# google/yggdrasil-decision-forests

Measured on NVIDIA H100. Metric: GBT boosting iters/sec, 10M rows x 200 num feats, higher is better.
Workload: dtype int64 fixed-point sums (q24 gradients), f64 split scores

## Files before the change

### include/ygg_b200.h

```cpp
#ifndef YGG_B200_H_
#define YGG_B200_H_

#include <stdint.h>

#ifdef __cplusplus
extern "C" {
#endif

#define YGG_ABI_VERSION 3

enum ygg_status {
  YGG_OK = 0,
  YGG_ERR_INVALID_ARGUMENT = 1,
  YGG_ERR_NO_DEVICE = 2,
  YGG_ERR_CUDA = 3,
  YGG_ERR_UNIMPLEMENTED = 4,
  YGG_ERR_CANCELLED = 5,
  YGG_ERR_IO = 6
};

enum ygg_loss {
  YGG_LOSS_BINOMIAL_LOG_LIKELIHOOD = 0,
  YGG_LOSS_SQUARED_ERROR = 1,
  YGG_LOSS_MULTINOMIAL_LOG_LIKELIHOOD = 2
// ... 150 lines not shown
int ygg_num_candidate_attributes(int32_t num_features, int32_t loss, int32_t num_candidate_attributes,
                                 float num_candidate_attributes_ratio, int32_t* k);
uint64_t ygg_candidate_key(uint32_t random_seed, int32_t tree, int32_t node, int32_t feature);
int ygg_gbt_set_candidate_sampling(ygg_gbt* h, int32_t num_candidate_attributes, float num_candidate_attributes_ratio);

int ygg_gbt_set_dart(ygg_gbt* h, float dropout_rate);
int ygg_gbt_get_dart_weights(ygg_gbt* h, float* out, int32_t capacity, int32_t* n);
int ygg_gbt_get_dart_dropped(ygg_gbt* h, int32_t iter, int32_t* out, int32_t capacity, int32_t* n);

int ygg_gbt_get_tree(ygg_gbt* h, int32_t iter, ygg_node* out, int32_t capacity, int32_t* n_nodes);
int ygg_gbt_get_category_set(ygg_gbt* h, int32_t iter, int32_t node, uint32_t* words, int32_t capacity, int32_t* n_words);
int ygg_gbt_train_loss(ygg_gbt* h, int32_t iter, float* loss, float* secondary);
int ygg_gbt_get_predictions(ygg_gbt* h, float* out, int64_t n);
int ygg_gbt_predict(ygg_gbt* h, const ygg_dataset* ds, float* out, int64_t n);

int ygg_gbt_set_predictions(ygg_gbt* h, const float* pred, int64_t n);

int ygg_tree_train_on_gradients(ygg_gbt* h, const float* gradients, const float* hessians,
                                ygg_node* out, int32_t capacity, int32_t* n_nodes);

enum ygg_hist_mode {
  YGG_HIST_ROOT_SUM = 0,
  YGG_HIST_PACKED = 1,
  YGG_HIST_SHARED = 2,
  YGG_HIST_HIST2 = 3,
  YGG_HIST_SEGMENTED = 4,
};
typedef struct ygg_hist_plan {
  int32_t mode;
  int32_t group;
  union {
    int32_t hist2_tiles;
    int32_t root_lanes;
  };
  int32_t chunk_blocks;
  int32_t slot_window;
  int32_t grid;
} ygg_hist_plan;
int ygg_debug_hist_plan(const ygg_gbt* h, int32_t level, ygg_hist_plan* out);
int ygg_debug_level_histogram(ygg_gbt* h, int32_t level, const ygg_hist_plan* plan, const float* gradients,
                              const float* second, const int32_t* slot_of_row, int32_t n_slots, uint64_t* out_sum,
                              uint32_t* out_cnt, uint64_t* out_second, float* out_scales);

int ygg_debug_wide_histogram(ygg_gbt* h, int32_t n_slots, uint64_t* out_sum, uint32_t* out_cnt, uint64_t* out_second);

int ygg_debug_capture_candidates(ygg_gbt* h, int32_t enabled);
typedef struct ygg_level_node {
  int32_t node;
  int32_t candidate;
  int32_t derived;
  int32_t reserved;
  int64_t num_examples;
} ygg_level_node;
typedef struct ygg_candidate {
  int32_t found;
  float score;
  int32_t threshold_bin;
  int32_t lo, hi;
  int32_t num_pos_examples;
  float threshold_value;
  uint32_t cat_mask[8];
} ygg_candidate;
int ygg_debug_level_candidates(ygg_gbt* h, int32_t level, int32_t capacity, ygg_level_node* nodes, ygg_candidate* cands,
                               uint32_t* sets, int32_t set_words, int32_t* n_nodes, float* scales);
int ygg_debug_level_tried(ygg_gbt* h, int32_t level, int32_t capacity, uint8_t* tried, int32_t* first_node, int32_t* n_nodes);

// ... 15 lines not shown
```

### yggdrasil-decision-forests_b200/_capi.py

```python
import ctypes as C
import os

import numpy as np

from . import _build

_LIB = None


class YggError(RuntimeError):
    def __init__(self, code, msg):
        super().__init__(f"[ygg status {code}] {msg}")
        self.code = code


class GbtConfig(C.Structure):
    _fields_ = [
        ("abi_version", C.c_int32), ("loss", C.c_int32), ("num_trees", C.c_int32),
        ("shrinkage", C.c_float), ("max_depth", C.c_int32), ("min_examples", C.c_int32),
        ("in_split_min_examples_check", C.c_int32), ("use_hessian_gain", C.c_int32),
        ("l1_regularization", C.c_float), ("l2_regularization", C.c_float),
        ("l2_regularization_categorical", C.c_float), ("clamp_leaf_logit", C.c_float),
        ("hessian_split_score_subtract_parent", C.c_int32), ("random_seed", C.c_uint32),
        ("subsample", C.c_float), ("validation_ratio", C.c_float),
# ... 2 lines not shown
        ("num_classes", C.c_int32), ("candidate_shuffle", C.c_int32), ("rng_words_consumed", C.c_uint32),
        ("split_jobs_draw_seeds", C.c_int32), ("growing_strategy", C.c_int32), ("max_num_nodes", C.c_int32),
        ("goss_alpha", C.c_float), ("goss_beta", C.c_float),
    ]


NODE_DTYPE = np.dtype([
    ("feature", "<i4"), ("threshold_bin", "<i4"), ("na_value", "<i4"), ("depth", "<i4"),
    ("neg_child", "<i4"), ("pos_child", "<i4"), ("split_score", "<f4"), ("leaf_value", "<f4"),
    ("num_examples", "<i8"), ("num_pos_examples", "<i8"), ("stat", "<f8", (3,)),
    ("condition_type", "<i4"), ("threshold_value", "<f4"), ("cat_mask", "<u4", (8,)),
])
assert NODE_DTYPE.itemsize == 112

FEATURE_DISCRETIZED_NUMERICAL = 0
FEATURE_CATEGORICAL = 1
FEATURE_NUMERICAL = 2

LEVEL_NODE_DTYPE = np.dtype([("node", "<i4"), ("candidate", "<i4"), ("derived", "<i4"), ("reserved", "<i4"),
                             ("num_examples", "<i8")])
assert LEVEL_NODE_DTYPE.itemsize == 24
CANDIDATE_DTYPE = np.dtype([("found", "<i4"), ("score", "<f4"), ("threshold_bin", "<i4"), ("lo", "<i4"), ("hi", "<i4"),
                            ("num_pos_examples", "<i4"), ("threshold_value", "<f4"), ("cat_mask", "<u4", (8,))])
assert CANDIDATE_DTYPE.itemsize == 60

HIST_ROOT_SUM, HIST_PACKED, HIST_SHARED, HIST2, HIST_SEGMENTED = 0, 1, 2, 3, 4


class HistPlan(C.Structure):
    _fields_ = [("mode", C.c_int32), ("group", C.c_int32), ("hist2_tiles", C.c_int32), ("chunk_blocks", C.c_int32),
                ("slot_window", C.c_int32), ("grid", C.c_int32)]

    root_lanes = property(lambda self: self.hist2_tiles, lambda self, v: setattr(self, "hist2_tiles", v))

    def __repr__(self):
        return "HistPlan(%s)" % ", ".join("%s=%d" % (k, getattr(self, k)) for k, _ in self._fields_)

ALLGATHER_FN = C.CFUNCTYPE(C.c_int, C.c_void_p, C.c_void_p, C.c_void_p, C.c_int64, C.c_void_p)
ALLREDUCE_FN = C.CFUNCTYPE(C.c_int, C.c_void_p, C.c_void_p, C.c_int64, C.c_int32, C.c_int32, C.c_void_p)
REDUCESCATTER_FN = C.CFUNCTYPE(C.c_int, C.c_void_p, C.c_void_p, C.c_int64, C.c_int32, C.c_int32, C.c_void_p)

EXPORTS = [
    "ygg_abi_version", "ygg_last_error", "ygg_device_count", "ygg_dataset_create",
    "ygg_dataset_set_feature_types", "ygg_dataset_destroy", "ygg_dataset_num_rows", "ygg_dataset_num_features",
    "ygg_gbt_config_init", "ygg_gbt_create", "ygg_gbt_destroy", "ygg_gbt_set_labels_i32",
    "ygg_gbt_set_labels_f32", "ygg_gbt_set_weights_f32", "ygg_gbt_set_validation_weights_f32", "ygg_gbt_set_feature_shard", "ygg_gbt_set_row_shard", "ygg_gbt_set_row_shard_scatter", "ygg_feature_shard",
    "ygg_merge_shard_best", "ygg_gbt_initial_prediction",
    "ygg_gbt_train", "ygg_gbt_train_timed", "ygg_gbt_step", "ygg_gbt_sync", "ygg_gbt_num_trees", "ygg_gbt_get_tree",
    "ygg_gbt_train_loss", "ygg_gbt_get_predictions", "ygg_gbt_set_predictions", "ygg_gbt_predict",
    "ygg_tree_train_on_gradients", "ygg_debug_hist_plan", "ygg_debug_level_histogram", "ygg_partition_rows",
    "ygg_gbt_set_profiling", "ygg_gbt_get_profile", "ygg_gbt_save_ydf",
    "ygg_discretize_boundaries", "ygg_discretize_encode", "ygg_model_write_ydf",
    "ygg_validation_split_mask", "ygg_dataset_split_rows", "ygg_gbt_set_validation_i32",
    "ygg_gbt_set_validation_f32", "ygg_gbt_validation_loss", "ygg_gbt_num_iterations", "ygg_gbt_final_validation",
    "ygg_gen_discretized_boundaries", "ygg_dataset_builder_create", "ygg_dataset_builder_add_numerical",
    "ygg_dataset_builder_add_numerical_async", "ygg_dataset_builder_get_numerical",
    "ygg_dataset_builder_add_bins", "ygg_dataset_builder_finish", "ygg_dataset_builder_destroy",
    "ygg_dataset_get_bins", "ygg_dataset_set_bucket_values", "ygg_gbt_tie_stats", "ygg_gbt_set_tie_rng_position",
    "ygg_gbt_best_split_window_bytes", "ygg_gbt_set_best_split_window", "ygg_comm_window_create",
    "ygg_comm_unique_id", "ygg_comm_create", "ygg_comm_destroy", "ygg_comm_allreduce", "ygg_comm_allgather", "ygg_comm_reducescatter",
    "ygg_dataset_set_wide_column", "ygg_dataset_get_wide_column", "ygg_debug_wide_histogram",
    "ygg_dataset_set_wide_categorical_column", "ygg_gbt_get_category_set",
    "ygg_dataset_set_numerical_column", "ygg_dataset_get_numerical_column",
    "ygg_debug_capture_candidates", "ygg_debug_level_candidates",
    "ygg_num_candidate_attributes", "ygg_candidate_key", "ygg_gbt_set_candidate_sampling", "ygg_debug_level_tried",
    "ygg_gbt_set_dart", "ygg_gbt_get_dart_weights", "ygg_gbt_get_dart_dropped",
# ... 737 lines not shown
```

### yggdrasil-decision-forests_b200/csrc/ygg_engine.cu

```cuda
#include <algorithm>
#include <mutex>
#include <random>
#include <cmath>
#include <cstdarg>
#include <cstdio>
#include <cstdlib>
#include <cstring>
#include <limits>
#include <map>
#include <queue>
#include <string>
#include <thread>
#include <vector>

#include <cuda_runtime.h>
#include <cub/device/device_radix_sort.cuh>
#include <cub/device/device_scan.cuh>
#include <nvtx3/nvToolsExt.h>

#include "../../include/ygg_b200.h"
#include "ygg_internal.h"
#include "../../include/ygg_b200_model.h"
#include "ygg_kernels.cuh"
#include "ygg_wide.cuh"
// ... 64 lines not shown
  return YGG_OK;
}
template <typename T>
int dev_alloc_plain(T** p, size_t count) {
  YGG_CUDA(cudaMalloc(reinterpret_cast<void**>(p), std::max<size_t>(count, 1) * sizeof(T)));
  return YGG_OK;
}
inline void dev_free(void* p) {
  if (p != nullptr) cudaFreeAsync(p, nullptr);
}

struct ProfileSlot {
  double ms = 0;
  int64_t launches = 0;
};

}


struct LossRec {
  double loss_sum;
  unsigned long long correct;
};

enum ShardMode { kShardNone = 0, kShardFeatures = 1, kShardRows = 2 };

struct HistLaunch {
  int mode;
  int G, S;
  int chunk, grid;
  int window, passes;
  int FL, T;
  int SL;
  int RL;
};

struct ygg_gbt {
  ygg_dataset* ds = nullptr;
  ygg_gbt_config cfg{};
  cudaStream_t stream = nullptr;
  bool has_labels = false;
  uint8_t* d_label_u8 = nullptr;
  float* d_label_f32 = nullptr;
  float initial_prediction = 0.f;
  float* d_pred = nullptr;
  float* d_g = nullptr;
  float* d_h = nullptr;
  uint32_t* d_q24 = nullptr;
  uint32_t* d_hq24 = nullptr;
  uint2* d_act = nullptr;
  uint32_t* d_act_h = nullptr;
  int32_t* d_act_count = nullptr;
  int32_t* d_act_sub = nullptr;
  uint32_t* d_root_cnt = nullptr;
  bool root_cnt_valid = false;
  int n_blocks = 0;
  uint16_t* d_node_of_row = nullptr;
  DeviceState* d_st = nullptr;
  LevelDesc* d_levels = nullptr;
  Family* d_fam[2] = {nullptr, nullptr};
  int32_t* d_slot_node[2] = {nullptr, nullptr};
  NodeRec* d_nodes_all = nullptr;
  NodeRec* d_nodes_scratch = nullptr;
  int tree_capacity = 0;
  unsigned long long* d_hist_sum[2] = {nullptr, nullptr};
  uint32_t* d_hist_cnt[2] = {nullptr, nullptr};
// ... 304 lines not shown
    YGG_RETURN_IF_ERROR(check_launch("k_sub_counts"));
  }
  uint32_t* d_max = *d_sub + static_cast<size_t>(n_subs) * f_count * kMaxBins;
  YGG_CUDA(cudaMemset(d_max, 0, sizeof(uint32_t)));
  const int subs_per_chunk = chunk_blocks / kSubBlocks;
  const int n_chunks = (n_subs + subs_per_chunk - 1) / subs_per_chunk;
  k_chunk_max<<<dim3(n_chunks, f_count), 256>>>(*d_sub, n_subs, subs_per_chunk, d_max);
  YGG_CUDA(cudaMemcpy(out_max, d_max, sizeof(uint32_t), cudaMemcpyDeviceToHost));
  return YGG_OK;
}

int raise_hist_smem_caps_once(int device) {
  static std::mutex mu;
  static std::vector<char> done;
  std::lock_guard<std::mutex> lock(mu);
  if (static_cast<int>(done.size()) <= device) done.resize(device + 1, 0);
  if (done[device]) return YGG_OK;
  size_t budget = 0;
  YGG_RETURN_IF_ERROR(hist_smem_budget(device, &budget));
  auto set_cap = [](size_t bytes) {
    return [bytes](auto kern) -> int {
      YGG_CUDA(cudaFuncSetAttribute(kern, cudaFuncAttributeMaxDynamicSharedMemorySize, static_cast<int>(bytes)));
      return YGG_OK;
    };
  };
  for (const bool hess : {false, true})
    for (const int mode : {kHistRootSum, kHistPacked, kHistShared})
      for (const bool multi : {false, true}) YGG_RETURN_IF_ERROR(for_hist_kernel(hess, mode, set_cap(budget), multi));
  const auto cap2 = set_cap(kHist2SmemBudget);
  YGG_RETURN_IF_ERROR(cap2(k_hist2<32, true>)); YGG_RETURN_IF_ERROR(cap2(k_hist2<32, false>));
  YGG_RETURN_IF_ERROR(cap2(k_hist2<16, true>)); YGG_RETURN_IF_ERROR(cap2(k_hist2<16, false>));
  YGG_RETURN_IF_ERROR(cap2(k_hist2<8, true>)); YGG_RETURN_IF_ERROR(cap2(k_hist2<8, false>));
  YGG_RETURN_IF_ERROR(set_cap(seg_smem_bytes(64))(k_hist_seg<32, 2>));
  YGG_RETURN_IF_ERROR(set_cap(seg_smem_bytes(32))(k_hist_seg<32, 1>));
  YGG_RETURN_IF_ERROR(set_cap(seg_smem_bytes(16))(k_hist_seg<16, 1>));
  YGG_RETURN_IF_ERROR(set_cap(seg_smem_bytes(8))(k_hist_seg<8, 1>));
  YGG_CUDA(cudaFuncSetAttribute(k_hist_seg<32, 2>, cudaFuncAttributePreferredSharedMemoryCarveout, cudaSharedmemCarveoutMaxShared));
  YGG_CUDA(cudaFuncSetAttribute(k_hist_seg<32, 1>, cudaFuncAttributePreferredSharedMemoryCarveout, cudaSharedmemCarveoutMaxShared));
  YGG_CUDA(cudaFuncSetAttribute(k_hist_seg<16, 1>, cudaFuncAttributePreferredSharedMemoryCarveout, cudaSharedmemCarveoutMaxShared));
  YGG_CUDA(cudaFuncSetAttribute(k_hist_seg<8, 1>, cudaFuncAttributePreferredSharedMemoryCarveout, cudaSharedmemCarveoutMaxShared));
  YGG_RETURN_IF_ERROR(set_cap(kRootSmemBytes)(k_hist_root_rows));
  done[device] = 1;
  return YGG_OK;
}

int configure_launches(ygg_gbt* h) {
  (void)cudaGetLastError();
  const bool hh = hist_hess(h);
  size_t budget = 0;
  YGG_RETURN_IF_ERROR(hist_smem_budget(h->ds->device, &budget));
  YGG_RETURN_IF_ERROR(raise_hist_smem_caps_once(h->ds->device));
  const int f_count = h->hist_f_end - h->hist_f_begin;
  const int n_blocks = static_cast<int>(h->ds->n_pad / kBlockRows);
  const int kSubBlocks = sub_blocks_of(h);
  const double min_items = 1.0, min_items2 = 0.9;
  auto choose_chunk = [&](int n_fgroups, int grid, int step, double need) {
    const int max_c = std::max(step, kHistMaxChunkBlocks / step * step);
    const int min_chunks = std::max(1, (n_blocks + max_c - 1) / max_c);
    int best = max_c;
    double best_score = -1;
    for (int nc = min_chunks; nc <= std::max(min_chunks, n_blocks); nc++) {
      const int c = std::min(max_c, ((n_blocks + nc - 1) / nc + step - 1) / step * step);
      const int real_nc = (n_blocks + c - 1) / c;
      const double per_cta = static_cast<double>(real_nc) * n_fgroups / grid;
      if (per_cta > 8.0 && nc > min_chunks) break;
      const double fill = static_cast<double>(n_blocks) / (static_cast<double>(real_nc) * c);
      const double eff = per_cta / std::ceil(per_cta) * fill;
      const double score = eff + (per_cta >= need ? 0.08 : 0.0);
      if (score > best_score + 1e-9) { best_score = score; best = c; }
    }
// ... 6 lines not shown
  for (int l = 0; l < h->num_levels; l++) {
    HistLaunch& pl = h->hist_plan[l];
    pl.mode = hh ? kHistShared : (l == 0 && !sampling(h)) ? kHistRootSum : kHistPacked;
    int S = level_slot_bound(h, l);
    pl.window = 0;
    pl.passes = 1;
    if (hist_smem_bytes(1, S, hh, pl.mode) > budget) {
      if (S > 254)
        return set_error(YGG_ERR_UNIMPLEMENTED, "max_depth=%d needs %d histogram slots at level %d; the active lists carry 8-bit slots",
                         h->cfg.max_depth, S, l);
      int s_pass = 1;
      while (hist_smem_bytes(1, 2 * s_pass + 1, hh, pl.mode) <= budget) s_pass *= 2;
      pl.window = s_pass;
      pl.passes = (S + s_pass - 1) / s_pass;
      S = s_pass + 1;
    }
    int G = 1;
    while (G < 8 && G < f_count && hist_smem_bytes(G + 1, S, hh, pl.mode) <= budget) G++;
    pl.G = G;
    pl.S = S;
    pl.grid = h->ds->num_sms;
    pl.FL = pl.T = 0;
    if (want_hist2 && !hh && S <= 2 && (l > 0 || pl.mode == kHistRootSum)) {
      int FL = 32;
      while (FL > 8 && FL / 2 >= 4 * n_groups) FL /= 2;
      int T = 2;
      if (hist2_smem_bytes(FL, S, T, l == 0) > kHist2SmemBudget) T = 1;
      if (hist2_smem_bytes(FL, S, T, l == 0) <= kHist2SmemBudget) { pl.FL = FL; pl.T = T; }
    }
    const bool packed = pl.mode == kHistPacked || (pl.FL > 0 && l > 0);
    const int n_fgroups = pl.FL > 0 ? (n_groups + pl.FL / 4 - 1) / (pl.FL / 4) : (f_count + G - 1) / G;
    pl.chunk = choose_chunk(n_fgroups, pl.grid, packed ? kSubBlocks : 1, pl.FL > 0 ? min_items2 : min_items);
    pl.SL = 0;
    pl.RL = 0;
    khist_plan[l] = pl;
    const int S_level = level_slot_bound(h, l);
    if (!hh && l > 0 && pl.mode == kHistPacked && pl.FL == 0 && S_level >= seg_min_slots(f_count, h->ds->n)) {
      int SL = 32;
      while (SL > 8 && SL / 2 >= f_count) SL /= 2;
      pl.SL = SL;
      pl.G = 1;
      pl.S = S_level;
      pl.window = 0;
      pl.passes = 1;
      pl.grid = h->ds->num_sms * kSegMinBlocks;
      pl.chunk = std::min(std::max(kSubBlocks, kHistMaxChunkBlocks / kSubBlocks * kSubBlocks),
                          (n_blocks + kSubBlocks - 1) / kSubBlocks * kSubBlocks);
    }
  }
  {
    std::map<int, uint32_t> max_of_chunk;
    uint32_t* d_sub = nullptr;
    int status = YGG_OK;
    for (int l = 0; l < h->num_levels && status == YGG_OK; l++) {
      HistLaunch& pl = h->hist_plan[l];
      if (pl.mode != kHistPacked && (pl.FL == 0 || l == 0)) continue;
      int chunk = pl.chunk;
      while (chunk >= kSubBlocks) {
        auto it = max_of_chunk.find(chunk);
        if (it == max_of_chunk.end()) {
          uint32_t m = 0;
          status = chunk_max_count(h, chunk, &d_sub, &m);
          if (status != YGG_OK) break;
          it = max_of_chunk.emplace(chunk, m).first;
        }
        if (it->second <= kPackedMaxUpdates) break;
        const int smaller = static_cast<int>(static_cast<double>(chunk) * 0.9 * kPackedMaxUpdates / it->second) / kSubBlocks * kSubBlocks;
        const int next = std::min(smaller, chunk - kSubBlocks);
        chunk = (next < kSubBlocks && chunk > kSubBlocks) ? kSubBlocks : next;
      }
      if (chunk < kSubBlocks) {
        if (pl.SL > 0) pl = khist_plan[l];
        pl.mode = kHistShared;
// ... 322 lines not shown
  h->d_hseg = nullptr; h->d_hseg_blk = nullptr; h->d_hseg_off = nullptr; h->d_hseg_piece = nullptr; h->d_hseg_meta = nullptr;
  h->d_hseg_temp = nullptr;
  h->hseg_temp_bytes = 0;
}
int ensure_seg_buffers(ygg_gbt* h) {
  if (h->d_hseg_temp != nullptr) return YGG_OK;
  const size_t ranges = static_cast<size_t>(kSegMaxSlots) * h->n_blocks;
  auto alloc_all = [&]() -> int {
    YGG_RETURN_IF_ERROR(dev_alloc(&h->d_hseg, static_cast<size_t>(h->ds->n_pad)));
    YGG_RETURN_IF_ERROR(dev_alloc(&h->d_hseg_blk, ranges));
    YGG_RETURN_IF_ERROR(dev_alloc(&h->d_hseg_off, ranges + 1));
    YGG_RETURN_IF_ERROR(dev_alloc(&h->d_hseg_piece, ranges + 1));
    YGG_RETURN_IF_ERROR(dev_alloc(&h->d_hseg_meta, 4));
    size_t temp_bytes = 0;
    YGG_CUDA(cub::DeviceScan::InclusiveSum(nullptr, temp_bytes, h->d_hseg_blk, h->d_hseg_blk, static_cast<int>(ranges)));
    char* temp = nullptr;
    YGG_RETURN_IF_ERROR(dev_alloc(&temp, temp_bytes));
    h->hseg_temp_bytes = temp_bytes;
    h->d_hseg_temp = temp;
    return YGG_OK;
  };
  const int st = alloc_all();
  if (st != YGG_OK) free_seg_buffers(h);
  return st;
}

int launch_hist_seg(ygg_gbt* h, int l, const LevelBuf& lb, const LevelDesc* levels, const HistLaunch& pl) {
  ygg_dataset* ds = h->ds;
  YGG_RETURN_IF_ERROR(ensure_bins_rows(ds));
  YGG_RETURN_IF_ERROR(ensure_seg_buffers(h));
  const int f_count = h->hist_f_end - h->hist_f_begin;
  const int n_chunks = (h->n_blocks + pl.chunk - 1) / pl.chunk;
  const int fpl = seg_lane_features(pl.SL, f_count);
  const int n_fg = seg_feature_groups(pl.SL, fpl, h->hist_f_begin, f_count);
  const int target_pieces = std::max(1, (kSegItemsPerCta * pl.grid + n_fg - 1) / n_fg);
  k_seg_count<<<std::min(h->n_blocks, ds->num_sms * 8), 256, 0, h->stream>>>(h->d_act, h->d_act_count, h->n_blocks, pl.S,
                                                                               levels, l, h->d_hseg_blk);
  YGG_RETURN_IF_ERROR(check_launch("k_seg_count"));
  YGG_CUDA(cub::DeviceScan::InclusiveSum(h->d_hseg_temp, h->hseg_temp_bytes, h->d_hseg_blk, h->d_hseg_blk, pl.S * h->n_blocks,
                                         h->stream));
  k_seg_ranges<<<1, kSegScanThreads, 0, h->stream>>>(h->d_hseg_blk, pl.S, h->n_blocks, pl.chunk, n_chunks, target_pieces,
                                                     h->d_hseg_off, h->d_hseg_piece, h->d_hseg_meta);
  YGG_RETURN_IF_ERROR(check_launch("k_seg_ranges"));
  k_seg_scatter<<<std::min(h->n_blocks, ds->num_sms * 8), 256, 0, h->stream>>>(h->d_act, h->d_act_count, h->n_blocks, pl.S, levels, l,
                                                               h->d_hseg_blk, h->d_hseg);
  YGG_RETURN_IF_ERROR(check_launch("k_seg_scatter"));
  SegParams sp{};
  sp.rows = ds->d_bins_rows; sp.row_bytes = static_cast<uint32_t>(seg_row_bytes(ds->F));
  sp.seg = h->d_hseg; sp.seg_off = h->d_hseg_off; sp.piece_start = h->d_hseg_piece; sp.meta = h->d_hseg_meta;
  sp.n_ranges = pl.S * n_chunks; sp.n_chunks = n_chunks;
  sp.f_begin = h->hist_f_begin; sp.f_count = f_count;
  sp.hist_sum = lb.sum; sp.hist_cnt = lb.cnt;
  sp.f_chunk = lb.f_chunk; sp.chunk_stride = static_cast<long long>(lb.chunk_u64);
  const size_t smem = seg_smem_bytes(pl.SL * fpl);
  if (fpl == 2) k_hist_seg<32, 2><<<pl.grid, kSegThreads, smem, h->stream>>>(sp);
  else if (pl.SL == 32) k_hist_seg<32, 1><<<pl.grid, kSegThreads, smem, h->stream>>>(sp);
  else if (pl.SL == 16) k_hist_seg<16, 1><<<pl.grid, kSegThreads, smem, h->stream>>>(sp);
  else k_hist_seg<8, 1><<<pl.grid, kSegThreads, smem, h->stream>>>(sp);
  h->launches_total += 5;
  return check_launch("k_hist_seg");
}

int launch_hist_root_rows(ygg_gbt* h, const LevelBuf& lb, const HistLaunch& pl) {
  ygg_dataset* ds = h->ds;
  YGG_RETURN_IF_ERROR(ensure_bins_rows(ds));
  RootRowsParams rp{};
  rp.rows = ds->d_bins_rows; rp.row_bytes = static_cast<uint32_t>(seg_row_bytes(ds->F));
  rp.q24 = h->d_q24; rp.act_count = h->d_act_count; rp.n_blocks = h->n_blocks; rp.chunk_blocks = pl.chunk;
  rp.f_begin = h->hist_f_begin; rp.f_count = h->hist_f_end - h->hist_f_begin;
  rp.hist_sum = lb.sum; rp.f_chunk = lb.f_chunk; rp.chunk_stride = static_cast<long long>(lb.chunk_u64);
  k_hist_root_rows<<<pl.grid, kRootThreads, kRootSmemBytes, h->stream>>>(rp);
  h->launches_total++;
  return check_launch("k_hist_root_rows");
}

int ensure_root_counts(ygg_gbt* h) {
  if (h->root_cnt_valid) return YGG_OK;
  const int f_count = h->hist_f_end - h->hist_f_begin;
  if (h->d_root_cnt) dev_free(h->d_root_cnt);
  h->d_root_cnt = nullptr;
  const LevelBuf lb = level_buf(h, 1, 1);
  const size_t padded = static_cast<size_t>(lb.W) * lb.f_chunk * kMaxBins;
  YGG_RETURN_IF_ERROR(dev_alloc(&h->d_root_cnt, padded));
  YGG_CUDA(cudaMemsetAsync(h->d_root_cnt, 0, padded * sizeof(uint32_t), h->stream));
  dim3 grid(std::max(1, h->ds->num_sms * 8 / std::max(1, f_count)), f_count);
  k_root_counts<<<grid, 256, 0, h->stream>>>(h->ds->d_bins, h->ds->n, h->ds->n_pad, f_count, h->hist_f_begin, h->d_root_cnt);
  h->launches_total++;
  YGG_RETURN_IF_ERROR(check_launch("k_root_counts"));
// ... 2444 lines not shown
  YGG_CUDA(cudaSetDevice(h->ds->device));
  (void)cudaGetLastError();
  YGG_RETURN_IF_ERROR(apply_pending(h));
  const int64_t n = h->ds->n;
  YGG_CUDA(cudaMemcpyAsync(h->d_g, gradients, n * sizeof(float), cudaMemcpyHostToDevice, h->stream));
  if (has_h(h)) YGG_CUDA(cudaMemcpyAsync(h->d_h, hessians, n * sizeof(float), cudaMemcpyHostToDevice, h->stream));
  const int root_candidate = (n >= h->cfg.min_examples && 1 < h->cfg.max_depth) ? 1 : 0;
  k_begin_iteration<<<1, 1, 0, h->stream>>>(h->d_st, h->d_levels, h->d_fam[0], h->d_slot_node[0], root_candidate);
  h->launches_total++;
  k_absmax<<<elementwise_grid(h), 256, 0, h->stream>>>(h->d_g, n, h->d_st);
  h->launches_total++;
  YGG_RETURN_IF_ERROR(check_launch("k_absmax"));
  h->scratch_tree = false;
  YGG_RETURN_IF_ERROR(grow_tree(h, h->d_nodes_scratch));
  if (h->cfg.growing_strategy == 1) YGG_RETURN_IF_ERROR(best_first_prune(h, h->d_nodes_scratch));
  YGG_RETURN_IF_ERROR(check_device_error(h));
  h->scratch_tree = true;
  std::vector<ygg_node> flat;
  YGG_RETURN_IF_ERROR(fetch_tree(h, h->d_nodes_scratch, &flat, true));
  *n_nodes = static_cast<int32_t>(flat.size());
  if (static_cast<int32_t>(flat.size()) > capacity) return set_error(YGG_ERR_INVALID_ARGUMENT, "capacity %d < %zu nodes", capacity, flat.size());
  std::memcpy(out, flat.data(), flat.size() * sizeof(ygg_node));
  return YGG_OK;
}

int ygg_debug_hist_plan(const ygg_gbt* h, int32_t level, ygg_hist_plan* out) {
  if (!h || !out) return set_error(YGG_ERR_INVALID_ARGUMENT, "null argument");
  if (level < 0 || level >= h->num_levels) return set_error(YGG_ERR_INVALID_ARGUMENT, "level %d outside [0, %d)", level, h->num_levels);
  const HistLaunch& pl = h->hist_plan[level];
  ygg_hist_plan p{};
  if (pl.FL > 0) {
    p.mode = YGG_HIST_HIST2; p.group = pl.FL; p.hist2_tiles = pl.T;
  } else if (pl.SL > 0) {
    p.mode = YGG_HIST_SEGMENTED; p.group = pl.SL;
  } else {
    p.mode = pl.mode == kHistRootSum ? YGG_HIST_ROOT_SUM : pl.mode == kHistPacked ? YGG_HIST_PACKED : YGG_HIST_SHARED;
    p.group = pl.G;
    p.root_lanes = pl.RL;
  }
  p.chunk_blocks = pl.chunk;
  p.slot_window = pl.window;
  p.grid = pl.grid;
  *out = p;
  return YGG_OK;
}

int ygg_debug_level_histogram(ygg_gbt* h, int32_t level, const ygg_hist_plan* plan, const float* gradients,
                              const float* second, const int32_t* slot_of_row, int32_t n_slots, uint64_t* out_sum,
                              uint32_t* out_cnt, uint64_t* out_second, float* out_scales) {
  if (!h || !gradients || !slot_of_row || !out_sum || !out_cnt || !out_scales) return set_error(YGG_ERR_INVALID_ARGUMENT, "null argument");
  if (level < 0 || level >= h->num_levels) return set_error(YGG_ERR_INVALID_ARGUMENT, "level %d outside [0, %d)", level, h->num_levels);
  if (n_slots < 1 || n_slots > 254) return set_error(YGG_ERR_INVALID_ARGUMENT, "n_slots=%d outside [1, 254] (8-bit slots)", n_slots);
  const bool hh = hist_hess(h);
  if (hh != (second != nullptr) || hh != (out_second != nullptr))
    return set_error(YGG_ERR_INVALID_ARGUMENT, hh ? "this handle keeps a second histogram plane: `second` and `out_second` are required"
                                                  : "this handle keeps no second histogram plane: `second` and `out_second` must be NULL");
  const float v_pow2 = hh ? (weighted(h) ? h->w_pow2 : h_pow2_of(h)) : 0.f;
  const int64_t n = h->ds->n;
  bool all_slot0 = true;
  for (int64_t r = 0; r < n; r++) {
    if (!std::isfinite(gradients[r])) return set_error(YGG_ERR_INVALID_ARGUMENT, "gradient of row %lld is not finite", static_cast<long long>(r));
    if (hh && !(second[r] >= 0.f && second[r] <= v_pow2))
      return set_error(YGG_ERR_INVALID_ARGUMENT, "second-plane value of row %lld outside [0, %g]", static_cast<long long>(r), v_pow2);
    if (slot_of_row[r] < -1 || slot_of_row[r] >= n_slots)
      return set_error(YGG_ERR_INVALID_ARGUMENT, "slot %d of row %lld outside [-1, %d)", slot_of_row[r], static_cast<long long>(r), n_slots);
    all_slot0 &= slot_of_row[r] == 0;
  }
  HistLaunch pl{};
  if (plan == nullptr) {
    pl = h->hist_plan[level];
    if (n_slots > level_slot_bound(h, level))
      return set_error(YGG_ERR_INVALID_ARGUMENT, "the plan of level %d holds %d slots, %d requested", level, level_slot_bound(h, level), n_slots);
  } else {
    const ygg_hist_plan& p = *plan;
    if (p.mode < YGG_HIST_ROOT_SUM || p.mode > YGG_HIST_SEGMENTED) return set_error(YGG_ERR_INVALID_ARGUMENT, "unknown mode %d", p.mode);
    const bool root_rows = p.mode == YGG_HIST_ROOT_SUM && p.root_lanes != 0;
    if (root_rows && p.root_lanes != kRootLanes)
      return set_error(YGG_ERR_INVALID_ARGUMENT, "root_lanes=%d: 0 (k_hist) or %d (k_hist_root_rows)", p.root_lanes, kRootLanes);
    const int max_chunk = root_rows ? kRootRowsMaxChunkBlocks : kHistMaxChunkBlocks;
    if (p.chunk_blocks < 1 || p.chunk_blocks > max_chunk)
      return set_error(YGG_ERR_INVALID_ARGUMENT, "chunk_blocks=%d outside [1, %d]", p.chunk_blocks, max_chunk);
    if (p.grid < 1 || p.grid > 65535) return set_error(YGG_ERR_INVALID_ARGUMENT, "grid=%d outside [1, 65535]", p.grid);
    if (p.slot_window < 0) return set_error(YGG_ERR_INVALID_ARGUMENT, "slot_window=%d", p.slot_window);
    pl.chunk = p.chunk_blocks; pl.grid = p.grid;
    if (p.mode == YGG_HIST_HIST2) {
      if (p.group != 8 && p.group != 16 && p.group != 32) return set_error(YGG_ERR_INVALID_ARGUMENT, "k_hist2: %d feature lanes (8, 16 or 32)", p.group);
      if (p.hist2_tiles != 1 && p.hist2_tiles != 2) return set_error(YGG_ERR_INVALID_ARGUMENT, "k_hist2: %d sub-tiles (1 or 2)", p.hist2_tiles);
      if (p.slot_window != 0) return set_error(YGG_ERR_INVALID_ARGUMENT, "k_hist2 has no multi-pass form");
      if (n_slots > 2) return set_error(YGG_ERR_INVALID_ARGUMENT, "k_hist2 with %d slots (at most 2)", n_slots);
      if (hist2_smem_bytes(p.group, n_slots, p.hist2_tiles, level == 0) > kHist2SmemBudget)
        return set_error(YGG_ERR_INVALID_ARGUMENT, "k_hist2 needs %zu bytes of shared memory (budget 216 KB)", hist2_smem_bytes(p.group, n_slots, p.hist2_tiles, level == 0));
      pl.FL = p.group; pl.T = p.hist2_tiles; pl.S = n_slots; pl.G = 1; pl.passes = 1;
      pl.mode = level == 0 ? kHistRootSum : kHistPacked;
    } else if (p.mode == YGG_HIST_SEGMENTED) {
      if (level == 0) return set_error(YGG_ERR_INVALID_ARGUMENT, "k_hist_seg runs below the root only");
      if (hh) return set_error(YGG_ERR_INVALID_ARGUMENT, "a second histogram plane is accumulated by the shared layout only");
      if (p.group != 8 && p.group != 16 && p.group != 32) return set_error(YGG_ERR_INVALID_ARGUMENT, "k_hist_seg: %d feature lanes (8, 16 or 32)", p.group);
      if (p.slot_window != 0) return set_error(YGG_ERR_INVALID_ARGUMENT, "k_hist_seg has no multi-pass form");
      pl.SL = p.group; pl.S = n_slots; pl.G = 1; pl.passes = 1;
      pl.mode = kHistPacked;
    } else if (root_rows) {
      if (p.group != kRootFpl) return set_error(YGG_ERR_INVALID_ARGUMENT, "k_hist_root_rows: group=%d features per lane (%d)", p.group, kRootFpl);
      if (p.slot_window != 0) return set_error(YGG_ERR_INVALID_ARGUMENT, "the root layout has no multi-pass form");
      pl.RL = p.root_lanes; pl.G = p.group; pl.S = n_slots; pl.passes = 1;
      pl.mode = kHistRootSum;
    } else {
      if (p.group < 1 || p.group > 8) return set_error(YGG_ERR_INVALID_ARGUMENT, "k_hist: group=%d outside [1, 8]", p.group);
      pl.mode = p.mode == YGG_HIST_ROOT_SUM ? kHistRootSum : p.mode == YGG_HIST_PACKED ? kHistPacked : kHistShared;
      pl.G = p.group;
      if (p.slot_window > 0) {
        if (pl.mode == kHistRootSum) return set_error(YGG_ERR_INVALID_ARGUMENT, "the root layout has no multi-pass form");
        pl.window = p.slot_window; pl.S = p.slot_window + 1; pl.passes = (n_slots + p.slot_window - 1) / p.slot_window;
      } else {
        pl.S = n_slots; pl.passes = 1;
      }
      size_t budget = 0;
      YGG_RETURN_IF_ERROR(hist_smem_budget(h->ds->device, &budget));
      if (hist_smem_bytes(pl.G, pl.S, hh, pl.mode) > budget)
        return set_error(YGG_ERR_INVALID_ARGUMENT, "k_hist with G=%d and %d slots per pass needs %zu bytes of shared memory (budget %zu)",
                         pl.G, pl.S, hist_smem_bytes(pl.G, pl.S, hh, pl.mode), budget);
    }
  }
  if (hh && (pl.FL > 0 || pl.SL > 0 || pl.RL > 0 || pl.mode != kHistShared))
    return set_error(YGG_ERR_INVALID_ARGUMENT, "a second histogram plane is accumulated by the shared layout only");
  if (pl.mode == kHistRootSum && (level != 0 || sampling(h) || !all_slot0 || n_slots != 1))
    return set_error(YGG_ERR_INVALID_ARGUMENT, "the root layouts need level 0, no row sampling and every row in slot 0");
  if (h->wide_total > 0 && n_slots > h->wide_slots)
    return set_error(YGG_ERR_INVALID_ARGUMENT, "the wide-column planes of this handle hold %d slots, %d requested", h->wide_slots, n_slots);
  YGG_CUDA(cudaSetDevice(h->ds->device));
  (void)cudaGetLastError();
  if (pl.mode == kHistPacked) {
    const int sub = sub_blocks_of(h);
// ... 530 lines not shown
```

### yggdrasil-decision-forests_b200/csrc/ygg_hist_seg.cuh

```cuda
#pragma once
#include <cstdint>
#include <type_traits>
#include <cub/block/block_scan.cuh>
#include <cuda_runtime.h>

#include "ygg_device.cuh"
#include "ygg_hist.cuh"

namespace ygg {

constexpr int kSegThreads = 1024;
constexpr int kSegMinBlocks = 1;
constexpr int kSegMinSlots = 4;
constexpr int kSegShallowMinFeatures = 128;
constexpr long long kSegShallowMinElements = 1000000000LL;
constexpr int kSegItemsPerCta = 4;
constexpr int kSegMinPiece = 4096;
constexpr int kSegMaxSlots = 256;
constexpr int kSegScanThreads = 512;

inline int seg_lane_features(int FL, int f_count) { return FL == 32 && f_count > 32 ? 2 : 1; }
inline int seg_min_slots(int f_count, long long rows) {
  return f_count >= kSegShallowMinFeatures && rows * f_count >= kSegShallowMinElements ? 1 : kSegMinSlots;
}
__host__ __device__ inline size_t seg_smem_bytes(int FI) { return static_cast<size_t>(kMaxBins) * 2 * FI * 4; }
__host__ __device__ inline int seg_feature_groups(int FL, int FPL, int f_begin, int f_count) {
  const int off = f_begin & (FPL - 1);
  return (f_count + off + FL * FPL - 1) / (FL * FPL);
}
inline int seg_row_bytes(int F) {
  int b = 32;
  while (b < F && b < 256) b *= 2;
  return b >= F ? b : (F + 255) / 256 * 256;
}

__global__ void __launch_bounds__(256) k_bins_to_rows(const uint8_t* bins, int64_t n_pad, int F, int row_bytes, uint8_t* rows) {
  const int64_t r = static_cast<int64_t>(blockIdx.x) * 256 + threadIdx.x;
  const int f0 = blockIdx.y * 32;
  if (r >= n_pad) return;
  uint32_t w[8] = {0u, 0u, 0u, 0u, 0u, 0u, 0u, 0u};
#pragma unroll
  for (int k = 0; k < 32; k++) {
    const int f = f0 + k;
    const uint32_t v = f < F ? bins[static_cast<int64_t>(f) * n_pad + r] : 0u;
    w[k >> 2] |= v << (8 * (k & 3));
  }
  uint4* dst = reinterpret_cast<uint4*>(rows + r * row_bytes + f0);
  dst[0] = make_uint4(w[0], w[1], w[2], w[3]);
  dst[1] = make_uint4(w[4], w[5], w[6], w[7]);
}

__device__ __forceinline__ uint32_t seg_slot_of(uint2 e, bool valid, uint32_t ns) {
  const uint32_t slot = e.x >> 24;
  return (valid && slot < ns) ? slot : 0xFFFFFFFFu;
}

__global__ void __launch_bounds__(256) k_seg_count(const uint2* act, const int32_t* act_count, int n_blocks, int S,
                                                   const LevelDesc* levels, int level, long long* blk) {
  __shared__ int c[kSegMaxSlots];
  const uint32_t ns = static_cast<uint32_t>(min(S, levels[level].num_slots));
  const int lane = threadIdx.x & 31;
  for (int b = blockIdx.x; b < n_blocks; b += gridDim.x) {
// ... 90 lines not shown
      if (slot != 0xFFFFFFFFu) o = cur[warp][slot];
      __syncwarp();
      if (slot != 0xFFFFFFFFu && rank == 0) cur[warp][slot] = o + __popc(mask);
      __syncwarp();
      if (slot != 0xFFFFFFFFu) seg[o + rank] = make_uint2(e.x, row0 + e.y);
    }
    __syncthreads();
  }
}

template <int FPL>
__device__ __forceinline__ uint32_t ldg_row(const uint8_t* p) {
  uint32_t v;
  if constexpr (FPL == 2) asm("ld.global.nc.L2::256B.u16 %0, [%1];" : "=r"(v) : "l"(p));
  else asm("ld.global.nc.L2::256B.u8 %0, [%1];" : "=r"(v) : "l"(p));
  return v;
}

struct SegParams {
  const uint8_t* rows;
  uint32_t row_bytes;
  const uint2* seg;
  const long long* seg_off;
  const int32_t* piece_start;
  int32_t* meta;
  int n_ranges, n_chunks;
  int f_begin, f_count;
  unsigned long long* hist_sum;
  uint32_t* hist_cnt;
  int f_chunk;
  long long chunk_stride;
};

template <int FL, int FPL>
__global__ void __launch_bounds__(kSegThreads, kSegMinBlocks) k_hist_seg(SegParams p) {
  static_assert(FL == 8 || FL == 16 || FL == 32, "feature lanes");
  static_assert(FPL == 1 || (FPL == 2 && FL == 32), "two features per lane at 32 lanes only");
  constexpr int FI = FL * FPL;
  constexpr int R = 32 / FL;
  constexpr int kSteps = 32 / R;
  constexpr int kInFlight = FL == 32 ? 32 : 8;
  constexpr int kWarps = kSegThreads / 32;
  constexpr int kWords = kMaxBins * 2 * FI;
  constexpr uint32_t kBinBytes = 2u * FI * 4u, kPlaneBytes = FI * 4u, kHalfBytes = FL * 4u;
  extern __shared__ __align__(16) uint32_t s_bins[];
  __shared__ int s_item;
  const int tid = threadIdx.x, lane = tid & 31, warp = tid >> 5;
  const int fl = lane % FL, sub = lane / FL;
  uint32_t s_base = static_cast<uint32_t>(__cvta_generic_to_shared(s_bins));
  asm volatile("mov.u32 %0, %0;" : "+r"(s_base));
  const int off = FPL == 2 ? (p.f_begin & 1) : 0;
  const int n_fg = seg_feature_groups(FL, FPL, p.f_begin, p.f_count);
  const int P = p.meta[0];
  const int n_items = p.meta[1] * n_fg;
  for (int i = tid; i < kWords; i += kSegThreads) s_bins[i] = 0u;
  const uint32_t a_lane = s_base + static_cast<uint32_t>(fl) * 4u;
  for (;;) {
    if (tid == 0) s_item = atomicAdd(&p.meta[2], 1);
    __syncthreads();
    const int item = s_item;
    if (item >= n_items) break;
    const int piece = item / n_fg, fg = item - piece * n_fg;
    int lo = 0, hi = p.n_ranges;
    while (hi - lo > 1) {
      const int mid = (lo + hi) >> 1;
      if (__ldg(p.piece_start + mid) <= piece) lo = mid;
      else hi = mid;
    }
    const long long beg = __ldg(p.seg_off + lo) + static_cast<long long>(piece - __ldg(p.piece_start + lo)) * P;
    const int len = static_cast<int>(min(static_cast<long long>(P), __ldg(p.seg_off + lo + 1) - beg));
    const int slot = lo / p.n_chunks;
    const int f0 = fg * FI - off;
    const int last = min(FI, p.f_count - f0) - 1;
    const uint8_t* col = p.rows + p.f_begin + f0 + min(fl * FPL, last & ~(FPL - 1));
    const uint2* sp = p.seg + beg;

    int e = warp * 32;
    uint2 cur = e + lane < len ? __ldg(sp + e + lane) : make_uint2(0u, 0u);
    for (; e < len; e += kWarps * 32) {
      const int en = e + kWarps * 32 + lane;
      const uint2 nxt = en < len ? __ldg(sp + en) : make_uint2(0u, 0u);
      const uint32_t xq = e + lane < len ? ((cur.x & kQMax) | 0x80000000u) : 0u;
#pragma unroll
      for (int j0 = 0; j0 < kSteps; j0 += kInFlight) {
        uint32_t b[kInFlight];
#pragma unroll
        for (int j = 0; j < kInFlight; j++) {
          const uint32_t row = __shfl_sync(0xFFFFFFFFu, cur.y, (j0 + j) * R + sub);
          b[j] = ldg_row<FPL>(col + static_cast<size_t>(row) * p.row_bytes);
        }
#pragma unroll
        for (int j = 0; j < kInFlight; j++) {
          const uint32_t x = __shfl_sync(0xFFFFFFFFu, xq, (j0 + j) * R + sub);
          const uint32_t inc = (((x >> kPackedCoarseShift) & 0x3Fu) << kPackedCntBits) | (x >> 31), q = x & kQMax;
          const uint32_t a = a_lane + (FPL == 2 ? b[j] & 0xFFu : b[j]) * kBinBytes;
          smem_red(a, inc);
          smem_red(a + kPlaneBytes, q);
          if constexpr (FPL == 2) {
            const uint32_t a1 = a_lane + kHalfBytes + (b[j] >> 8) * kBinBytes;
            smem_red(a1, inc);
            smem_red(a1 + kPlaneBytes, q);
          }
        }
      }
      cur = nxt;
    }
    __syncthreads();

    constexpr int QL = FI >= 16 ? 4 : 2;
    constexpr int TB = 32 / QL;
    constexpr int kQuadGroups = FI / (4 * QL);
    constexpr int kTiles = kMaxBins / TB * kQuadGroups;
    const int tr = lane / QL, tq = lane % QL;
    for (int t = warp; t < kTiles; t += kWarps) {
      const int bin = t / kQuadGroups * TB + tr;
      const int k0 = (t % kQuadGroups * QL + tq) * 4;
      uint4* w = reinterpret_cast<uint4*>(s_bins + bin * 2 * FI + k0);
      const uint4 c4 = w[0], l4 = w[FI / 4];
      w[0] = make_uint4(0u, 0u, 0u, 0u);
      w[FI / 4] = make_uint4(0u, 0u, 0u, 0u);
      const uint32_t cs[4] = {c4.x, c4.y, c4.z, c4.w}, ls[4] = {l4.x, l4.y, l4.z, l4.w};
#pragma unroll
      for (int j = 0; j < 4; j++) {
        const int k = k0 + j;
        const int f = f0 + (k % FL) * FPL + k / FL;
        const uint32_t c = cs[j];
        if (c == 0u || f < 0 || f >= p.f_count) continue;
        size_t oc;
        const size_t o = slot_hist_offset(slot, f, bin, p.f_chunk, p.chunk_stride, &oc);
        const unsigned long long base = static_cast<unsigned long long>(c >> kPackedCntBits) << kPackedCoarseShift;
        atomicAdd(&p.hist_sum[o], base + static_cast<uint32_t>(ls[j] - static_cast<uint32_t>(base)));
        atomicAdd(&p.hist_cnt[oc], c & kPackedMaxUpdates);
      }
    }
  }
}

}
```

Measured before the change: 169.3.

## Fold narrow trailing feature group into previous segmented histogram pass

When the last 64-feature group of the segmented histogram kernel holds at most 8 columns, that tail is no longer a separate work item. The preceding group's pass now also accumulates the tail, using an extra shared-memory histogram region where each lane handles a sub-row times tail-column pair. This removes one full sweep over the segment row lists and row gathers per piece. In exchange it adds shared memory per CTA, which may lower occupancy, and adds extra shuffle and load work inside the inner loop on the tail group.

```diff
diff --git a/include/ygg_b200.h b/include/ygg_b200.h
--- a/include/ygg_b200.h
+++ b/include/ygg_b200.h
@@ -206,6 +206,7 @@
   union {
     int32_t hist2_tiles;
     int32_t root_lanes;
+    int32_t seg_tail;
   };
   int32_t chunk_blocks;
   int32_t slot_window;
diff --git a/yggdrasil-decision-forests_b200/_capi.py b/yggdrasil-decision-forests_b200/_capi.py
--- a/yggdrasil-decision-forests_b200/_capi.py
+++ b/yggdrasil-decision-forests_b200/_capi.py
@@ -58,6 +58,7 @@
                 ("slot_window", C.c_int32), ("grid", C.c_int32)]
 
     root_lanes = property(lambda self: self.hist2_tiles, lambda self, v: setattr(self, "hist2_tiles", v))
+    seg_tail = property(lambda self: self.hist2_tiles, lambda self, v: setattr(self, "hist2_tiles", v))
 
     def __repr__(self):
         return "HistPlan(%s)" % ", ".join("%s=%d" % (k, getattr(self, k)) for k, _ in self._fields_)
diff --git a/yggdrasil-decision-forests_b200/csrc/ygg_engine.cu b/yggdrasil-decision-forests_b200/csrc/ygg_engine.cu
--- a/yggdrasil-decision-forests_b200/csrc/ygg_engine.cu
+++ b/yggdrasil-decision-forests_b200/csrc/ygg_engine.cu
@@ -120,6 +120,7 @@
   int window, passes;
   int FL, T;
   int SL;
+  int TW;
   int RL;
 };
 
@@ -490,10 +491,12 @@
   YGG_RETURN_IF_ERROR(cap2(k_hist2<16, true>)); YGG_RETURN_IF_ERROR(cap2(k_hist2<16, false>));
   YGG_RETURN_IF_ERROR(cap2(k_hist2<8, true>)); YGG_RETURN_IF_ERROR(cap2(k_hist2<8, false>));
   YGG_RETURN_IF_ERROR(set_cap(seg_smem_bytes(64))(k_hist_seg<32, 2>));
+  YGG_RETURN_IF_ERROR(set_cap(seg_smem_bytes(64) + seg_tail_smem_bytes(kSegTail))(k_hist_seg<32, 2, kSegTail>));
   YGG_RETURN_IF_ERROR(set_cap(seg_smem_bytes(32))(k_hist_seg<32, 1>));
   YGG_RETURN_IF_ERROR(set_cap(seg_smem_bytes(16))(k_hist_seg<16, 1>));
   YGG_RETURN_IF_ERROR(set_cap(seg_smem_bytes(8))(k_hist_seg<8, 1>));
   YGG_CUDA(cudaFuncSetAttribute(k_hist_seg<32, 2>, cudaFuncAttributePreferredSharedMemoryCarveout, cudaSharedmemCarveoutMaxShared));
+  YGG_CUDA(cudaFuncSetAttribute(k_hist_seg<32, 2, kSegTail>, cudaFuncAttributePreferredSharedMemoryCarveout, cudaSharedmemCarveoutMaxShared));
   YGG_CUDA(cudaFuncSetAttribute(k_hist_seg<32, 1>, cudaFuncAttributePreferredSharedMemoryCarveout, cudaSharedmemCarveoutMaxShared));
   YGG_CUDA(cudaFuncSetAttribute(k_hist_seg<16, 1>, cudaFuncAttributePreferredSharedMemoryCarveout, cudaSharedmemCarveoutMaxShared));
   YGG_CUDA(cudaFuncSetAttribute(k_hist_seg<8, 1>, cudaFuncAttributePreferredSharedMemoryCarveout, cudaSharedmemCarveoutMaxShared));
@@ -566,6 +569,7 @@
     const int n_fgroups = pl.FL > 0 ? (n_groups + pl.FL / 4 - 1) / (pl.FL / 4) : (f_count + G - 1) / G;
     pl.chunk = choose_chunk(n_fgroups, pl.grid, packed ? kSubBlocks : 1, pl.FL > 0 ? min_items2 : min_items);
     pl.SL = 0;
+    pl.TW = 0;
     pl.RL = 0;
     khist_plan[l] = pl;
     const int S_level = level_slot_bound(h, l);
@@ -573,6 +577,7 @@
       int SL = 32;
       while (SL > 8 && SL / 2 >= f_count) SL /= 2;
       pl.SL = SL;
+      pl.TW = SL == 32 ? seg_tail_width(h->hist_f_begin, f_count) : 0;
       pl.G = 1;
       pl.S = S_level;
       pl.window = 0;
@@ -961,7 +966,7 @@
   const int f_count = h->hist_f_end - h->hist_f_begin;
   const int n_chunks = (h->n_blocks + pl.chunk - 1) / pl.chunk;
   const int fpl = seg_lane_features(pl.SL, f_count);
-  const int n_fg = seg_feature_groups(pl.SL, fpl, h->hist_f_begin, f_count);
+  const int n_fg = seg_feature_groups(pl.SL, fpl, h->hist_f_begin, f_count) - (pl.TW > 0 ? 1 : 0);
   const int target_pieces = std::max(1, (kSegItemsPerCta * pl.grid + n_fg - 1) / n_fg);
   k_seg_count<<<std::min(h->n_blocks, ds->num_sms * 8), 256, 0, h->stream>>>(h->d_act, h->d_act_count, h->n_blocks, pl.S,
                                                                                levels, l, h->d_hseg_blk);
@@ -981,8 +986,9 @@
   sp.f_begin = h->hist_f_begin; sp.f_count = f_count;
   sp.hist_sum = lb.sum; sp.hist_cnt = lb.cnt;
   sp.f_chunk = lb.f_chunk; sp.chunk_stride = static_cast<long long>(lb.chunk_u64);
-  const size_t smem = seg_smem_bytes(pl.SL * fpl);
-  if (fpl == 2) k_hist_seg<32, 2><<<pl.grid, kSegThreads, smem, h->stream>>>(sp);
+  const size_t smem = seg_smem_bytes(pl.SL * fpl) + seg_tail_smem_bytes(pl.TW);
+  if (pl.TW > 0) k_hist_seg<32, 2, kSegTail><<<pl.grid, kSegThreads, smem, h->stream>>>(sp);
+  else if (fpl == 2) k_hist_seg<32, 2><<<pl.grid, kSegThreads, smem, h->stream>>>(sp);
   else if (pl.SL == 32) k_hist_seg<32, 1><<<pl.grid, kSegThreads, smem, h->stream>>>(sp);
   else if (pl.SL == 16) k_hist_seg<16, 1><<<pl.grid, kSegThreads, smem, h->stream>>>(sp);
   else k_hist_seg<8, 1><<<pl.grid, kSegThreads, smem, h->stream>>>(sp);
@@ -3493,7 +3499,7 @@
   if (pl.FL > 0) {
     p.mode = YGG_HIST_HIST2; p.group = pl.FL; p.hist2_tiles = pl.T;
   } else if (pl.SL > 0) {
-    p.mode = YGG_HIST_SEGMENTED; p.group = pl.SL;
+    p.mode = YGG_HIST_SEGMENTED; p.group = pl.SL; p.seg_tail = pl.TW;
   } else {
     p.mode = pl.mode == kHistRootSum ? YGG_HIST_ROOT_SUM : pl.mode == kHistPacked ? YGG_HIST_PACKED : YGG_HIST_SHARED;
     p.group = pl.G;
@@ -3558,7 +3564,10 @@
       if (hh) return set_error(YGG_ERR_INVALID_ARGUMENT, "a second histogram plane is accumulated by the shared layout only");
       if (p.group != 8 && p.group != 16 && p.group != 32) return set_error(YGG_ERR_INVALID_ARGUMENT, "k_hist_seg: %d feature lanes (8, 16 or 32)", p.group);
       if (p.slot_window != 0) return set_error(YGG_ERR_INVALID_ARGUMENT, "k_hist_seg has no multi-pass form");
-      pl.SL = p.group; pl.S = n_slots; pl.G = 1; pl.passes = 1;
+      const int tw = p.group == 32 ? seg_tail_width(h->hist_f_begin, h->hist_f_end - h->hist_f_begin) : 0;
+      if (p.seg_tail != 0 && p.seg_tail != tw)
+        return set_error(YGG_ERR_INVALID_ARGUMENT, "k_hist_seg: seg_tail=%d: 0 or this shard's tail width %d", p.seg_tail, tw);
+      pl.SL = p.group; pl.TW = p.seg_tail; pl.S = n_slots; pl.G = 1; pl.passes = 1;
       pl.mode = kHistPacked;
     } else if (root_rows) {
       if (p.group != kRootFpl) return set_error(YGG_ERR_INVALID_ARGUMENT, "k_hist_root_rows: group=%d features per lane (%d)", p.group, kRootFpl);
diff --git a/yggdrasil-decision-forests_b200/csrc/ygg_hist_seg.cuh b/yggdrasil-decision-forests_b200/csrc/ygg_hist_seg.cuh
--- a/yggdrasil-decision-forests_b200/csrc/ygg_hist_seg.cuh
+++ b/yggdrasil-decision-forests_b200/csrc/ygg_hist_seg.cuh
@@ -28,6 +28,14 @@
   const int off = f_begin & (FPL - 1);
   return (f_count + off + FL * FPL - 1) / (FL * FPL);
 }
+constexpr int kSegTail = 8;
+inline int seg_tail_width(int f_begin, int f_count) {
+  if (f_count <= 32) return 0;
+  const int n_fg = seg_feature_groups(32, 2, f_begin, f_count);
+  const int t = f_count + (f_begin & 1) - (n_fg - 1) * 64;
+  return n_fg >= 2 && t <= kSegTail ? kSegTail : 0;
+}
+__host__ __device__ inline size_t seg_tail_smem_bytes(int TW) { return TW > 0 ? static_cast<size_t>(kMaxBins) * 2 * 32 * 4 : 0; }
 inline int seg_row_bytes(int F) {
   int b = 32;
   while (b < F && b < 256) b *= 2;
@@ -184,10 +192,11 @@
   long long chunk_stride;
 };
 
-template <int FL, int FPL>
+template <int FL, int FPL, int TW = 0>
 __global__ void __launch_bounds__(kSegThreads, kSegMinBlocks) k_hist_seg(SegParams p) {
   static_assert(FL == 8 || FL == 16 || FL == 32, "feature lanes");
   static_assert(FPL == 1 || (FPL == 2 && FL == 32), "two features per lane at 32 lanes only");
+  static_assert(TW == 0 || (FPL == 2 && TW == kSegTail), "a folded tail of kSegTail columns, paired form only");
   constexpr int FI = FL * FPL;
   constexpr int R = 32 / FL;
   constexpr int kSteps = 32 / R;
@@ -195,6 +204,9 @@
   constexpr int kWarps = kSegThreads / 32;
   constexpr int kWords = kMaxBins * 2 * FI;
   constexpr uint32_t kBinBytes = 2u * FI * 4u, kPlaneBytes = FI * 4u, kHalfBytes = FL * 4u;
+  constexpr int TR = TW > 0 ? 32 / TW : 1;
+  constexpr int kTailLag = 12;
+  constexpr int kTailWords = TW > 0 ? kMaxBins * 2 * 32 : 0;
   extern __shared__ __align__(16) uint32_t s_bins[];
   __shared__ int s_item;
   const int tid = threadIdx.x, lane = tid & 31, warp = tid >> 5;
@@ -202,16 +214,15 @@
   uint32_t s_base = static_cast<uint32_t>(__cvta_generic_to_shared(s_bins));
   asm volatile("mov.u32 %0, %0;" : "+r"(s_base));
   const int off = FPL == 2 ? (p.f_begin & 1) : 0;
-  const int n_fg = seg_feature_groups(FL, FPL, p.f_begin, p.f_count);
-  const int P = p.meta[0];
-  const int n_items = p.meta[1] * n_fg;
-  for (int i = tid; i < kWords; i += kSegThreads) s_bins[i] = 0u;
+  const int n_fg = seg_feature_groups(FL, FPL, p.f_begin, p.f_count) - (TW > 0 ? 1 : 0);
+  for (int i = tid; i < kWords + kTailWords; i += kSegThreads) s_bins[i] = 0u;
   const uint32_t a_lane = s_base + static_cast<uint32_t>(fl) * 4u;
   for (;;) {
     if (tid == 0) s_item = atomicAdd(&p.meta[2], 1);
     __syncthreads();
     const int item = s_item;
-    if (item >= n_items) break;
+    if (item >= p.meta[1] * n_fg) break;
+    const int P = p.meta[0];
     const int piece = item / n_fg, fg = item - piece * n_fg;
     int lo = 0, hi = p.n_ranges;
     while (hi - lo > 1) {
@@ -226,36 +237,70 @@
     const int last = min(FI, p.f_count - f0) - 1;
     const uint8_t* col = p.rows + p.f_begin + f0 + min(fl * FPL, last & ~(FPL - 1));
     const uint2* sp = p.seg + beg;
-
-    int e = warp * 32;
-    uint2 cur = e + lane < len ? __ldg(sp + e + lane) : make_uint2(0u, 0u);
-    for (; e < len; e += kWarps * 32) {
-      const int en = e + kWarps * 32 + lane;
-      const uint2 nxt = en < len ? __ldg(sp + en) : make_uint2(0u, 0u);
-      const uint32_t xq = e + lane < len ? ((cur.x & kQMax) | 0x80000000u) : 0u;
-#pragma unroll
-      for (int j0 = 0; j0 < kSteps; j0 += kInFlight) {
-        uint32_t b[kInFlight];
-#pragma unroll
-        for (int j = 0; j < kInFlight; j++) {
-          const uint32_t row = __shfl_sync(0xFFFFFFFFu, cur.y, (j0 + j) * R + sub);
-          b[j] = ldg_row<FPL>(col + static_cast<size_t>(row) * p.row_bytes);
-        }
-#pragma unroll
-        for (int j = 0; j < kInFlight; j++) {
-          const uint32_t x = __shfl_sync(0xFFFFFFFFu, xq, (j0 + j) * R + sub);
-          const uint32_t inc = (((x >> kPackedCoarseShift) & 0x3Fu) << kPackedCntBits) | (x >> 31), q = x & kQMax;
-          const uint32_t a = a_lane + (FPL == 2 ? b[j] & 0xFFu : b[j]) * kBinBytes;
-          smem_red(a, inc);
-          smem_red(a + kPlaneBytes, q);
-          if constexpr (FPL == 2) {
-            const uint32_t a1 = a_lane + kHalfBytes + (b[j] >> 8) * kBinBytes;
-            smem_red(a1, inc);
-            smem_red(a1 + kPlaneBytes, q);
+    const bool tail = TW > 0 && fg == n_fg - 1;
+
+    {
+      int e = warp * 32;
+      uint2 cur = e + lane < len ? __ldg(sp + e + lane) : make_uint2(0u, 0u);
+      for (; e < len; e += kWarps * 32) {
+        const int en = e + kWarps * 32 + lane;
+        const uint2 nxt = en < len ? __ldg(sp + en) : make_uint2(0u, 0u);
+        const uint32_t xq = e + lane < len ? ((cur.x & kQMax) | 0x80000000u) : 0u;
+#pragma unroll
+        for (int j0 = 0; j0 < kSteps; j0 += kInFlight) {
+          uint32_t b[kInFlight];
+          uint32_t tb[TW > 0 ? TW : 1];
+#pragma unroll
+          for (int j = 0; j < kInFlight; j++) {
+            const uint32_t row = __shfl_sync(0xFFFFFFFFu, cur.y, (j0 + j) * R + sub);
+            b[j] = ldg_row<FPL>(col + static_cast<size_t>(row) * p.row_bytes);
+          }
+#pragma unroll
+          for (int j = 0; j < kInFlight; j++) {
+            const uint32_t x = __shfl_sync(0xFFFFFFFFu, xq, (j0 + j) * R + sub);
+            const uint32_t inc = (((x >> kPackedCoarseShift) & 0x3Fu) << kPackedCntBits) | (x >> 31), q = x & kQMax;
+            const uint32_t a = a_lane + (FPL == 2 ? b[j] & 0xFFu : b[j]) * kBinBytes;
+            smem_red(a, inc);
+            smem_red(a + kPlaneBytes, q);
+            if constexpr (FPL == 2) {
+              const uint32_t a1 = a_lane + kHalfBytes + (b[j] >> 8) * kBinBytes;
+              smem_red(a1, inc);
+              smem_red(a1 + kPlaneBytes, q);
+            }
+            if constexpr (TW > 0) {
+              const int t = j - kTailLag;
+              if (tail && t >= 0 && t < TW) {
+                uint32_t tl;
+                asm volatile("mov.u32 %0, %%laneid;" : "=r"(tl));
+                const int tr = tl / TW, tc = tl % TW;
+                const uint32_t row = __shfl_sync(0xFFFFFFFFu, cur.y, t * TR + tr);
+                tb[t] = 0u;
+                if (f0 + FI + tc < p.f_count) tb[t] = ldg_row<1>(col + static_cast<size_t>(row) * p.row_bytes + (FI + tc - 2 * static_cast<int>(tl)));
+              }
+            }
+          }
+          if constexpr (TW > 0) {
+            if (tail) {
+              uint32_t tl;
+              asm volatile("mov.u32 %0, %%laneid;" : "=r"(tl));
+              const int tr = tl / TW, tc = tl % TW;
+              const bool t_ok = f0 + FI + tc < p.f_count;
+              const uint32_t t_lane = a_lane + kWords * 4u;
+#pragma unroll
+              for (int t = 0; t < TW; t++) {
+                const uint32_t x = __shfl_sync(0xFFFFFFFFu, xq, t * TR + tr);
+                const uint32_t inc = (((x >> kPackedCoarseShift) & 0x3Fu) << kPackedCntBits) | (x >> 31), q = x & kQMax;
+                const uint32_t a = t_lane + tb[t] * (2u * 32u * 4u);
+                if (t_ok) {
+                  smem_red(a, inc);
+                  smem_red(a + 32u * 4u, q);
+                }
+              }
+            }
           }
         }
+        cur = nxt;
       }
-      cur = nxt;
     }
     __syncthreads();
 
@@ -285,7 +330,32 @@
         atomicAdd(&p.hist_cnt[oc], c & kPackedMaxUpdates);
       }
     }
-  }
-}
-
-}
+    if constexpr (TW > 0) {
+      const int tr = lane / TW, tc = lane % TW;
+      const int f = f0 + FI + tc;
+      if (tail && f < p.f_count) {
+        for (int bin = warp * TR + tr; bin < kMaxBins; bin += kWarps * TR) {
+          unsigned long long sum = 0ull;
+          uint32_t cnt = 0u;
+#pragma unroll
+          for (int k = 0; k < TR; k++) {
+            uint32_t* w = s_bins + kWords + bin * 2 * 32 + (tr + k) % TR * TW + tc;
+            const uint32_t c = w[0], l = w[32];
+            w[0] = 0u;
+            w[32] = 0u;
+            const unsigned long long base = static_cast<unsigned long long>(c >> kPackedCntBits) << kPackedCoarseShift;
+            sum += base + static_cast<uint32_t>(l - static_cast<uint32_t>(base));
+            cnt += c & kPackedMaxUpdates;
+          }
+          if (cnt == 0u) continue;
+          size_t oc;
+          const size_t o = slot_hist_offset(slot, f, bin, p.f_chunk, p.chunk_stride, &oc);
+          atomicAdd(&p.hist_sum[o], sum);
+          atomicAdd(&p.hist_cnt[oc], cnt);
+        }
+      }
+    }
+  }
+}
+
+}
```

New measurement: 175.3 (median of 6 runs). 1.04x the previous value.
